# victorramirez952/tomography_3d_reconstructor

Hardware: AMD Instinct MI355X
Metric: Mvoxels/s (SDF+MC) on 1024^3 ellipsoid stack; achieved HBM GB/s vs peak (higher is better)
Workload: dtype f64

## Files before the change

### include/tomo_hip.h

```cpp
#ifndef TOMO_HIP_H
#define TOMO_HIP_H

#include <stddef.h>
#include <stdint.h>

#ifdef __cplusplus
extern "C" {
#endif

#define TOMO_OK 0
#define TOMO_E_ARG (-1)
#define TOMO_E_LAUNCH (-2)
#define TOMO_E_SIZE (-3)
#define TOMO_E_WORKSPACE (-4)

int tomo_abi_version(void);
const char *tomo_error_string(int code);
int tomo_host_mc_cell(const float *h_v, double iso, int8_t *h_tris, int *h_uses_centre);
double tomo_host_mc_edge_offset(double va, double vb);
void tomo_host_mc_centre_offset(const double *h_v8, double *h_out3);

int tomo_host_checksum(const void *h_data, int64_t nbytes, int nthreads, uint64_t *h_out);
int tomo_host_checksum_impl(const void *h_data, int64_t nbytes, int nthreads, int impl, uint64_t *h_out);
int64_t tomo_host_checksum_chunk_bytes(void);
// ... 106 lines not shown
                   const double *xt, double r2, int level, int32_t *map, void *workspace, int64_t workspace_bytes, void *stream);
int tomo_edt_threshold_masked(const uint64_t *sites, int nz, int ny, int nx, const double *zt, const double *yt, const double *xt,
                              int inside, double r2, int keep_less, const uint64_t *mask, uint64_t *out, void *workspace,
                              int64_t workspace_bytes, void *stream);
int tomo_edt_thickness_finish(int32_t *map, const uint64_t *bits, int nz, int ny, int nx, const float *values, int levels,
                              int64_t *counts, void *stream);
int tomo_pack_threshold(const uint8_t *grey, uint64_t *bits, int nz, int ny, int nx, int threshold, void *stream);
int tomo_obj_write(const char *path, const void *vertices, int vertex_is_double, int64_t nv, const int64_t *faces,
                   int64_t nf, int nthreads);
int tomo_obj_block_format(int kind, const void *h_rows, int64_t n, int nthreads, void **h_block, int64_t *h_nbytes);
int tomo_obj_block_pwrite(const char *path, int64_t offset, const void *h_block);
void tomo_obj_block_free(void *h_block);

int tomo_extend_bits(const uint64_t *bits, uint64_t *ext, int nz, int ny, int nx, int pad, void *stream);
int tomo_field_fill(const uint64_t *ext, float *field, int nz, int ny, int nx, int pad, int gaussian,
                    unsigned long long *signs, uint8_t *gcls, void *stream);
int tomo_field_fill_bits(const uint64_t *bits, float *field, int nz, int ny, int nx, int pad, unsigned long long *signs,
                         uint8_t *gcls, void *stream);
int64_t tomo_field_span_bytes(int nz, int ny, int nx, int pad);
int tomo_field_fill_bits_sparse(const uint64_t *bits, float *field, int nz, int ny, int nx, int pad, unsigned long long *signs,
                                uint8_t *gcls, uint8_t *span_ws, void *stream);
int64_t tomo_sign_rows(int Ny);
int64_t tomo_sign_buffer_words(int Nz, int Ny, int Nx, int xorg);
int tomo_field_signs(const float *field, int Nz, int Ny, int Nx, int64_t pitch, int xorg, double iso, int z_begin,
                     int z_end, unsigned long long *signs, uint8_t *gcls, void *stream);

int tomo_mc_classify(const unsigned long long *signs, const uint8_t *gcls, int Nz, int Ny, int Nx, int xorg,
                     unsigned long long *seg_act, uint32_t *seg_cnt, void *stream);
int tomo_mc_scan_segments(const uint32_t *seg_cnt, int64_t nseg, uint32_t *seg_aoff, unsigned long long *totals,
                          void *workspace, int64_t workspace_bytes, void *stream);
int64_t tomo_mc_scan_workspace_bytes(int64_t n);
int tomo_mc_scan(const uint32_t *counts, int64_t n, uint32_t *off_a, uint32_t *off_b, uint32_t *nz_ids,
                 unsigned long long *totals, void *workspace, int64_t workspace_bytes, void *stream);
int tomo_mc_list(int Nz, int Ny, int Nx, int xorg, const uint32_t *seg_aoff, const unsigned long long *seg_act,
                 unsigned long long *vox_key, void *stream);
int tomo_mc_eval(const float *field, int Nz, int Ny, int Nx, int64_t pitch, int xorg, double iso,
                 const unsigned long long *vox_key, int64_t na, uint32_t *vox_counts, uint8_t *vox_flags, void *stream);
int tomo_mc_list_capped(int Nz, int Ny, int Nx, int xorg, const uint32_t *seg_aoff, const unsigned long long *seg_act,
                        unsigned long long *vox_key, int64_t cap, void *stream);
int tomo_mc_eval_capped(const float *field, int Nz, int Ny, int Nx, int64_t pitch, int xorg, double iso,
                        const unsigned long long *vox_key, int64_t cap, const unsigned long long *na_dev,
                        uint32_t *vox_counts, uint8_t *vox_flags, void *stream);
int tomo_mc_emit(const float *field, int Nz, int Ny, int Nx, int64_t pitch, int xorg, double iso,
                 const unsigned long long *vox_key, int64_t na, const unsigned long long *seg_act,
                 const uint32_t *seg_aoff, const uint32_t *vox_voff, const uint32_t *vox_foff, const uint8_t *vox_flags,
                 int z_offset, unsigned long long *vkey, float *vpos, int32_t *faces, unsigned long long *totals,
                 void *stream);

int tomo_mc_first_touch(const float *field, int Nz, int Ny, int Nx, int64_t pitch, int xorg, double iso,
                        const unsigned long long *vox_key, int64_t na, const unsigned long long *seg_act,
                        const uint32_t *seg_aoff, const uint32_t *vox_voff, const uint8_t *vox_flags, int mode,
                        uint32_t *created, const uint32_t *base, int32_t *ft_rank, unsigned long long *totals, void *stream);

int tomo_mc3_list(int Nz, int Ny, int Nx, int xorg, const uint32_t *seg_cnt, const unsigned long long *seg_act,
                  uint32_t *seg_blk, uint32_t *seg_aoff, unsigned long long *vox_key, int64_t cap, unsigned long long *tot,
                  void *stream);
int tomo_mc3_eval(const float *field, int Nz, int Ny, int Nx, int64_t pitch, int xorg, double iso,
                  const unsigned long long *vox_key, int64_t cap, const unsigned long long *tot, int z_offset,
                  uint32_t *vox_loc, int32_t *vox_til, uint8_t *vox_flags, uint16_t *vox_used, float *vox_f3, float *vox_c3,
                  uint32_t *blk3, void *stream);
int64_t tomo_mc3_slice_table_words(int Nz, int Ny);
int64_t tomo_mc3_sort_segments(int Nz, int Ny);
int tomo_mc3_scan(int Nz, int Ny, int Nx, int xorg, const uint32_t *seg_aoff, const uint32_t *vox_loc, int64_t cap,
                  uint32_t *blk3, uint32_t *slice_tab, unsigned long long *tot, int64_t cap_v, int64_t cap_f, void *stream);
int tomo_mc3_vertices(int Nz, int Ny, int Nx, int xorg, const unsigned long long *vox_key, int64_t cap,
                      const unsigned long long *tot, const uint32_t *vox_loc, const uint8_t *vox_flags, const float *vox_f3,
                      const float *vox_c3, const uint32_t *blk3, const uint32_t *slice_tab, int z_offset, int shift,
                      const double *cum, int64_t ncum, const double *adj, int64_t nadj, float mm_y, float mm_x, float *vrec,
                      uint32_t *keys, uint32_t *idx, void *stream);
int64_t tomo_mc3_sort_workspace_bytes(int64_t cap_v, int64_t nseg);
int tomo_mc3_sort_rank_top(const float *vrec, uint32_t *keys, uint32_t *idx, int64_t cap_v, int Nz, int Ny, const uint32_t *slice_tab,
                           unsigned long long *tot, float *uniq, int32_t *table, void *workspace, int64_t workspace_bytes,
                           float z_top, void *stream);
int tomo_mc3_sort_rank_fused(const float *vrec, const uint32_t *keys, int64_t cap_v, int Nz, int Ny, uint32_t *slice_tab,
                             unsigned long long *tot, float *uniq, int32_t *table, float z_top, void *stream);
int tomo_mc3_faces(int Nz, int Ny, int Nx, int xorg, const unsigned long long *vox_key, int64_t cap, unsigned long long *tot,
                   const unsigned long long *seg_act, const uint32_t *seg_aoff, const uint32_t *vox_loc, const int32_t *vox_til,
                   const uint16_t *vox_used, const uint32_t *blk3, const int32_t *table, int64_t *faces, int64_t cap_f,
                   void *stream);

int tomo_vertex_finalize(float *vpos, int64_t nv, int shift, const double *cum, int64_t ncum,
                         const double *adj, int64_t nadj, float mm_y, float mm_x, void *stream);
int64_t tomo_mesh_unique_workspace_bytes(int64_t nv);
int tomo_mesh_unique(const float *vpos, int64_t nv, float *uniq, int32_t *rank, unsigned long long *totals,
                     void *workspace, int64_t workspace_bytes, void *stream);
int tomo_mesh_lookup(const float *uniq, int64_t nu, const float *query, int64_t nq, int32_t *out,
                     unsigned long long *missing, void *stream);
int tomo_slab_top_rows(const float *uniq, const unsigned long long *tot, int64_t cap_v, int64_t cap, float *msg, void *stream);
int tomo_slab_lookup(const float *uniq, const unsigned long long *tot, int64_t cap_v, const float *msg, int64_t cap,
                     int32_t *out, unsigned long long *missing, void *stream);
int tomo_slab_summary(const unsigned long long *tot, int64_t cap_v, const float *msg_in, unsigned long long *missing,
                      int64_t cap_top, int64_t caller_flags, int64_t *out, void *stream);
int tomo_slab_lookup_summary(const float *uniq, const unsigned long long *tot, int64_t cap_v, const float *msg, int64_t cap,
                             int32_t *out, int64_t cap_top, int64_t caller_flags, unsigned long long *scratch, int64_t *summary,
                             void *stream);
int tomo_mc3_faces_slab(int Nz, int Ny, int Nx, int xorg, const unsigned long long *vox_key, int64_t cap, unsigned long long *tot,
                        const unsigned long long *seg_act, const uint32_t *seg_aoff, const uint32_t *vox_loc, const int32_t *vox_til,
                        const uint16_t *vox_used, const uint32_t *blk3, const int32_t *table, int64_t *faces, int64_t cap_f,
                        const int64_t *gathered, int rank, int world, const int32_t *ids_next, int64_t cap_top, int64_t cap_v,
                        void *stream);
int tomo_mesh_volume_area(const float *verts, const int64_t *faces, int64_t nf, double *out, void *stream);

int tomo_layer_colors(const void *verts, int is_f64, int64_t nv, int64_t stride, double start1, double end1, int enable1,
                      double start2, double end2, int enable2, uint8_t *rgba, void *stream);
int64_t tomo_mesh_edge_table_bytes(int64_t nf);
int tomo_mesh_edges(const int64_t *faces, int64_t nf, int64_t nv, void *table, int64_t table_bytes, unsigned long long *counters,
// ... 25 lines not shown
```

### tomography_3d_reconstructor_amd/_lib.py

```python
import ctypes
import os
import subprocess

_HERE = os.path.dirname(os.path.abspath(__file__))
SO_PATH = os.environ.get("TOMO_LIB") or os.path.join(_HERE, "libtomo_hip.so")
CSRC = os.path.join(_HERE, "csrc")

_c_i = ctypes.c_int
_c_i64 = ctypes.c_int64
_c_p = ctypes.c_void_p
_c_d = ctypes.c_double
_c_f = ctypes.c_float

SIGNATURES = {
    "tomo_abi_version": (_c_i, []),
    "tomo_error_string": (ctypes.c_char_p, [_c_i]),
    "tomo_host_mc_cell": (_c_i, [_c_p, _c_d, _c_p, _c_p]),
    "tomo_host_mc_edge_offset": (_c_d, [_c_d, _c_d]),
    "tomo_host_mc_centre_offset": (None, [_c_p, _c_p]),
    "tomo_host_checksum": (_c_i, [_c_p, _c_i64, _c_i, _c_p]),
    "tomo_host_checksum_impl": (_c_i, [_c_p, _c_i64, _c_i, _c_i, _c_p]),
    "tomo_host_checksum_chunk_bytes": (_c_i64, []),
    "tomo_host_checksum_part": (_c_i, [_c_p, _c_i64, _c_i64, _c_i, _c_i, _c_p]),
    "tomo_host_checksum_fold": (_c_i, [_c_p, _c_i64, _c_i64, _c_p]),
# ... 39 lines not shown
    "tomo_cc_seam_union": (_c_i, [_c_p, _c_i, _c_i, _c_i, _c_p, _c_i64, _c_p, _c_p, _c_p, _c_p, _c_p, _c_p, _c_i64, _c_i64, _c_i64, _c_p,
                                  _c_p, _c_p]),
    "tomo_cc_merge_tables": (_c_i, [_c_p, _c_i, _c_i64, _c_i64, _c_p, _c_i64, _c_i64, _c_i64, _c_p, _c_p, _c_p, _c_p, _c_p, _c_p]),
    "tomo_cc_local_maps": (_c_i, [_c_p, _c_p, _c_p, _c_p, _c_i64, _c_i64, _c_i64, _c_i64, _c_i, _c_p, _c_p, _c_p]),
    "tomo_cc_filter_map": (_c_i, [_c_p, _c_i, _c_i, _c_i, _c_p, _c_i64, _c_p, _c_p, _c_p, _c_p, _c_i64, _c_p, _c_p]),
    "tomo_cc_expand_map": (_c_i, [_c_p, _c_i, _c_i, _c_i, _c_p, _c_i64, _c_p, _c_p, _c_p, _c_p, _c_i64, _c_p, _c_p]),
    "tomo_edt_workspace_bytes": (_c_i64, [_c_i, _c_i, _c_i, _c_i64]),
    "tomo_edt_chunk_columns": (_c_i64, [_c_i, _c_i, _c_i, _c_i64]),
    "tomo_edt_distance": (_c_i, [_c_p, _c_i, _c_i, _c_i, _c_p, _c_p, _c_p, _c_i, _c_p, _c_p, _c_i64, _c_p]),
    "tomo_edt_threshold": (_c_i, [_c_p, _c_i, _c_i, _c_i, _c_p, _c_p, _c_p, _c_i, _c_d, _c_i, _c_p, _c_p, _c_i64, _c_p]),
    "tomo_edt_argmax": (_c_i, [_c_p, _c_i, _c_i, _c_i, _c_p, _c_p, _c_p, _c_i, _c_p, _c_p, _c_i64, _c_p]),
    "tomo_edt_squared": (_c_i, [_c_p, _c_i, _c_i, _c_i, _c_p, _c_p, _c_p, _c_i, _c_p, _c_p, _c_i64, _c_p]),
    "tomo_edt_at_least": (_c_i, [_c_p, _c_p, _c_i, _c_i, _c_i, _c_d, _c_p, _c_p]),
    "tomo_edt_cover": (_c_i, [_c_p, _c_p, _c_i, _c_i, _c_i, _c_p, _c_p, _c_p, _c_d, _c_i, _c_p, _c_p, _c_i64, _c_p]),
    "tomo_edt_threshold_masked": (_c_i, [_c_p, _c_i, _c_i, _c_i, _c_p, _c_p, _c_p, _c_i, _c_d, _c_i, _c_p, _c_p, _c_p, _c_i64, _c_p]),
    "tomo_edt_thickness_finish": (_c_i, [_c_p, _c_p, _c_i, _c_i, _c_i, _c_p, _c_i, _c_p, _c_p]),
    "tomo_pack_threshold": (_c_i, [_c_p, _c_p, _c_i, _c_i, _c_i, _c_i, _c_p]),
    "tomo_obj_write": (_c_i, [ctypes.c_char_p, _c_p, _c_i, _c_i64, _c_p, _c_i64, _c_i]),
    "tomo_obj_block_format": (_c_i, [_c_i, _c_p, _c_i64, _c_i, ctypes.POINTER(_c_p), ctypes.POINTER(_c_i64)]),
    "tomo_obj_block_pwrite": (_c_i, [ctypes.c_char_p, _c_i64, _c_p]),
    "tomo_obj_block_free": (None, [_c_p]),
    "tomo_fill_holes_slice": (_c_i, [_c_p, _c_i, _c_i, _c_i, _c_i, _c_p, _c_p]),
    "tomo_fill_holes_ends": (_c_i, [_c_p, _c_i, _c_i, _c_i, _c_p, _c_p]),
    "tomo_pack_close_ends": (_c_i, [_c_p, _c_p, _c_i, _c_i, _c_i, _c_p, _c_p]),
    "tomo_pack_bits_pair": (_c_i, [_c_p, _c_p, _c_i, _c_p, _c_p, _c_i, _c_i, _c_i, _c_p]),
    "tomo_slab_edges": (_c_i, [_c_p, _c_p, _c_i, _c_i, _c_i, _c_i, _c_p, _c_p, _c_i, _c_i, _c_p, _c_p, _c_p, _c_i, _c_p, _c_p, _c_p, _c_p,
                               _c_i, _c_p, _c_p]),
    "tomo_pack_close_range": (_c_i, [_c_p, _c_p, _c_i, _c_i, _c_i, _c_i, _c_i, _c_p, _c_p, _c_i, _c_i, _c_p]),
    "tomo_close_ends_workspace_words": (_c_i64, [_c_i, _c_i, _c_i]),
    "tomo_close_ends_scan": (_c_i, [_c_p, _c_i, _c_i, _c_i, _c_p, _c_p]),
    "tomo_close_ends_gp": (_c_i, [_c_p, _c_i, _c_i, _c_i, _c_p, _c_p, _c_p]),
    "tomo_morph_fused": (_c_i, [_c_p, _c_p, _c_i, _c_i, _c_i, ctypes.c_uint32, _c_i, _c_p]),
    "tomo_smooth": (_c_i, [_c_p, _c_p, _c_i, _c_i, _c_i, _c_i, _c_i, _c_p]),
    "tomo_extend_bits": (_c_i, [_c_p, _c_p, _c_i, _c_i, _c_i, _c_i, _c_p]),
    "tomo_field_fill": (_c_i, [_c_p, _c_p, _c_i, _c_i, _c_i, _c_i, _c_i, _c_p, _c_p, _c_p]),
    "tomo_field_fill_bits": (_c_i, [_c_p, _c_p, _c_i, _c_i, _c_i, _c_i, _c_p, _c_p, _c_p]),
    "tomo_field_span_bytes": (_c_i64, [_c_i, _c_i, _c_i, _c_i]),
    "tomo_field_fill_bits_sparse": (_c_i, [_c_p, _c_p, _c_i, _c_i, _c_i, _c_i, _c_p, _c_p, _c_p, _c_p]),
    "tomo_sign_rows": (_c_i64, [_c_i]),
    "tomo_sign_buffer_words": (_c_i64, [_c_i, _c_i, _c_i, _c_i]),
    "tomo_field_signs": (_c_i, [_c_p, _c_i, _c_i, _c_i, _c_i64, _c_i, _c_d, _c_i, _c_i, _c_p, _c_p, _c_p]),
    "tomo_mc_classify": (_c_i, [_c_p, _c_p, _c_i, _c_i, _c_i, _c_i, _c_p, _c_p, _c_p]),
    "tomo_mc_scan_segments": (_c_i, [_c_p, _c_i64, _c_p, _c_p, _c_p, _c_i64, _c_p]),
    "tomo_mc_scan_workspace_bytes": (_c_i64, [_c_i64]),
    "tomo_mc_scan": (_c_i, [_c_p, _c_i64, _c_p, _c_p, _c_p, _c_p, _c_p, _c_i64, _c_p]),
    "tomo_mc_list": (_c_i, [_c_i, _c_i, _c_i, _c_i, _c_p, _c_p, _c_p, _c_p]),
    "tomo_mc_eval": (_c_i, [_c_p, _c_i, _c_i, _c_i, _c_i64, _c_i, _c_d, _c_p, _c_i64, _c_p, _c_p, _c_p]),
    "tomo_mc_list_capped": (_c_i, [_c_i, _c_i, _c_i, _c_i, _c_p, _c_p, _c_p, _c_i64, _c_p]),
    "tomo_mc_eval_capped": (_c_i, [_c_p, _c_i, _c_i, _c_i, _c_i64, _c_i, _c_d, _c_p, _c_i64, _c_p, _c_p, _c_p, _c_p]),
    "tomo_mc_emit": (_c_i, [_c_p, _c_i, _c_i, _c_i, _c_i64, _c_i, _c_d, _c_p, _c_i64, _c_p, _c_p, _c_p, _c_p, _c_p, _c_i, _c_p,
                            _c_p, _c_p, _c_p, _c_p]),
    "tomo_mc_first_touch": (_c_i, [_c_p, _c_i, _c_i, _c_i, _c_i64, _c_i, _c_d, _c_p, _c_i64, _c_p, _c_p, _c_p, _c_p, _c_i, _c_p,
                                   _c_p, _c_p, _c_p, _c_p]),
    "tomo_mc3_list": (_c_i, [_c_i, _c_i, _c_i, _c_i, _c_p, _c_p, _c_p, _c_p, _c_p, _c_i64, _c_p, _c_p]),
    "tomo_mc3_eval": (_c_i, [_c_p, _c_i, _c_i, _c_i, _c_i64, _c_i, _c_d, _c_p, _c_i64, _c_p, _c_i, _c_p, _c_p, _c_p, _c_p, _c_p,
                             _c_p, _c_p, _c_p]),
    "tomo_mc3_slice_table_words": (_c_i64, [_c_i, _c_i]),
    "tomo_mc3_sort_segments": (_c_i64, [_c_i, _c_i]),
    "tomo_mc3_scan": (_c_i, [_c_i, _c_i, _c_i, _c_i, _c_p, _c_p, _c_i64, _c_p, _c_p, _c_p, _c_i64, _c_i64, _c_p]),
    "tomo_mc3_vertices": (_c_i, [_c_i, _c_i, _c_i, _c_i, _c_p, _c_i64, _c_p, _c_p, _c_p, _c_p, _c_p, _c_p, _c_p, _c_i, _c_i,
                                 _c_p, _c_i64, _c_p, _c_i64, _c_f, _c_f, _c_p, _c_p, _c_p, _c_p]),
    "tomo_mc3_sort_workspace_bytes": (_c_i64, [_c_i64, _c_i64]),
    "tomo_mc3_sort_rank_top": (_c_i, [_c_p, _c_p, _c_p, _c_i64, _c_i, _c_i, _c_p, _c_p, _c_p, _c_p, _c_p, _c_i64, _c_f, _c_p]),
    "tomo_mc3_sort_rank_fused": (_c_i, [_c_p, _c_p, _c_i64, _c_i, _c_i, _c_p, _c_p, _c_p, _c_p, _c_f, _c_p]),
    "tomo_mc3_faces": (_c_i, [_c_i, _c_i, _c_i, _c_i, _c_p, _c_i64, _c_p, _c_p, _c_p, _c_p, _c_p, _c_p, _c_p, _c_p, _c_p, _c_i64, _c_p]),
    "tomo_vertex_finalize": (_c_i, [_c_p, _c_i64, _c_i, _c_p, _c_i64, _c_p, _c_i64, _c_f, _c_f, _c_p]),
    "tomo_mesh_unique_workspace_bytes": (_c_i64, [_c_i64]),
    "tomo_mesh_unique": (_c_i, [_c_p, _c_i64, _c_p, _c_p, _c_p, _c_p, _c_i64, _c_p]),
    "tomo_mesh_lookup": (_c_i, [_c_p, _c_i64, _c_p, _c_i64, _c_p, _c_p, _c_p]),
    "tomo_slab_top_rows": (_c_i, [_c_p, _c_p, _c_i64, _c_i64, _c_p, _c_p]),
    "tomo_slab_lookup": (_c_i, [_c_p, _c_p, _c_i64, _c_p, _c_i64, _c_p, _c_p, _c_p]),
    "tomo_slab_summary": (_c_i, [_c_p, _c_i64, _c_p, _c_p, _c_i64, _c_i64, _c_p, _c_p]),
    "tomo_slab_lookup_summary": (_c_i, [_c_p, _c_p, _c_i64, _c_p, _c_i64, _c_p, _c_i64, _c_i64, _c_p, _c_p, _c_p]),
    "tomo_mc3_faces_slab": (_c_i, [_c_i, _c_i, _c_i, _c_i, _c_p, _c_i64, _c_p, _c_p, _c_p, _c_p, _c_p, _c_p, _c_p, _c_p, _c_p, _c_i64,
                                   _c_p, _c_i, _c_i, _c_p, _c_i64, _c_i64, _c_p]),
    "tomo_mesh_volume_area": (_c_i, [_c_p, _c_p, _c_i64, _c_p, _c_p]),
    "tomo_layer_colors": (_c_i, [_c_p, _c_i, _c_i64, _c_i64, _c_d, _c_d, _c_i, _c_d, _c_d, _c_i, _c_p, _c_p]),
    "tomo_mesh_edge_table_bytes": (_c_i64, [_c_i64]),
    "tomo_mesh_edges": (_c_i, [_c_p, _c_i64, _c_i64, _c_p, _c_i64, _c_p, _c_p]),
    "tomo_mesh_seam_edges": (_c_i, [_c_p, _c_i64, _c_i64, _c_i64, _c_p, _c_i64, _c_p, _c_p]),
    "tomo_mesh_seam_merge": (_c_i, [_c_p, _c_i64, _c_i64, _c_p, _c_i64, _c_p, _c_p]),
    "tomo_mesh_orient_workspace_bytes": (_c_i64, [_c_i64]),
    "tomo_mesh_orient": (_c_i, [_c_p, _c_i64, _c_i64, _c_p, _c_i64, _c_p, _c_p, _c_p]),
    "tomo_mesh_signed_volume": (_c_i, [_c_p, _c_p, _c_i64, _c_p, _c_p, _c_p]),
    "tomo_glb_pack_faces": (_c_i, [_c_p, _c_i64, _c_p, _c_p, _c_p, _c_i, _c_p]),
    "tomo_glb_pack_positions": (_c_i, [_c_p, _c_i, _c_i64, _c_p, _c_p, _c_p]),
    "tomo_mesh_vertex_normals_workspace_bytes": (_c_i64, [_c_i64, _c_i64]),
    "tomo_mesh_vertex_normals": (_c_i, [_c_p, _c_i64, _c_p, _c_i, _c_i64, _c_p, _c_i64, _c_p, _c_p, _c_p]),
    "tomo_mesh_vertex_normals_seeded": (_c_i, [_c_p, _c_i64, _c_p, _c_i, _c_i64, _c_p, _c_i64, _c_p, _c_p, _c_p, _c_i64, _c_p, _c_i64,
                                              _c_i, _c_p]),
}

_LIB = None


class TomoError(RuntimeError):
    pass


class TomoUnavailable(TomoError):
    """No MI355X visible / libtomo_hip.so not built.  The one failure the drop-in classes never turn into the
    reference's `return None`: there is no CPU fallback to hide behind."""


def build(force=False):
    srcs = [os.path.join(CSRC, f) for f in os.listdir(CSRC) if f.endswith((".hip", ".h", ".cpp", "Makefile"))]
# ... 30 lines not shown
```

### tomography_3d_reconstructor_amd/csrc/mc.hip

```cpp
#include <cstring>
#include <cstdlib>
#include "tomo_common.h"
#include <rocprim/rocprim.hpp>

#define MC_LUT_QUAL __device__ const
#define MC_FN __device__ static inline
#include "mc_cell.h"

#define SEG 256
#define KEY_XBITS 20
static_assert(KEY_XBITS + 2 == TOMO_KEY_ROW_SHIFT, "key layout shared with mesh.hip");

struct McGrid {
    int Nz, Ny, Nx;
    int64_t pitch;
    int xorg;
    int segs_per_row;
    double iso;
};

typedef float float4u __attribute__((ext_vector_type(4), aligned(4)));
typedef float float2u __attribute__((ext_vector_type(2), aligned(4)));
typedef float float3u __attribute__((ext_vector_type(3), aligned(4)));
typedef int int3u __attribute__((ext_vector_type(3), aligned(4)));
// ... 808 lines not shown
                                                           const u64 *__restrict__ vox_key, int64_t cap,
                                                           const u64 *__restrict__ tot, int z_offset,
                                                           u32 *__restrict__ vox_loc, int32_t *__restrict__ vox_til,
                                                           uint8_t *__restrict__ vox_flags, uint16_t *__restrict__ vox_used,
                                                           float *__restrict__ vox_f3, float *__restrict__ vox_c3,
                                                           u32 *__restrict__ blk3, int64_t nblk)
{
    __shared__ u32 wsum[4];
    const int lane = threadIdx.x & 63, w = threadIdx.x >> 6;
    const int64_t i = (int64_t)blockIdx.x * MC3_BLK + threadIdx.x;
    const u64 na = tot[0];
    const bool live = i < cap && (u64)i < na && na <= (u64)cap;
    u32 packed = 0;
    if (live) {
        Cell c;
        load_cell(field, g, vox_key[i], c);
        int ntri = 0;
        int32_t til = 0;
        u32 used = 0;
        if (c.cell_ok && c.index != 0 && c.index != 255) {
            const McTiling t = mc_cell_tiling(c.v, c.index);
            ntri = t.ntri;
            if (t.centre) c.flags |= 8;
            til = (int32_t)(((intptr_t)t.tris - (intptr_t)LUT_TILING1) * 16 + ntri);
            const int ix = c.index;
#define BICH(a, b) ((u32)(((ix >> (a)) ^ (ix >> (b))) & 1))
            used = BICH(0, 1) | BICH(1, 2) << 1 | BICH(2, 3) << 2 | BICH(3, 0) << 3 | BICH(4, 5) << 4 | BICH(5, 6) << 5 | BICH(6, 7) << 6 |
                   BICH(7, 4) << 7 | BICH(0, 4) << 8 | BICH(1, 5) << 9 | BICH(2, 6) << 10 | BICH(3, 7) << 11 | (t.centre ? 1u << 12 : 0u);
#undef BICH
            if (ntri == 0) used = 0;
        }
        const int Zg = c.Z + z_offset;
        float3u f3;
        f3.x = (float)((double)Zg + mc_edge_offset(c.v[0], c.v[4]));
        f3.y = (float)((double)c.Y + mc_edge_offset(c.v[0], c.v[3]));
        f3.z = (float)((double)c.X + mc_edge_offset(c.v[0], c.v[1]));
        *(float3u *)(vox_f3 + 3 * i) = f3;
        if (c.flags & 8) {
            double ox, oy, oz;
            mc_centre_offset(c.v, &ox, &oy, &oz);
            *(float3u *)(vox_c3 + 3 * i) = (float3u){(float)((double)Zg + oz), (float)((double)c.Y + oy), (float)((double)c.X + ox)};
        }
        vox_til[i] = til;
        vox_flags[i] = (uint8_t)c.flags;
        vox_used[i] = (uint16_t)used;
        packed = (u32)__popc(c.flags & 3) | ((u32)__popc(c.flags & 12) << 10) | ((u32)ntri << 20);
    }
    const u32 inc = wave_inclusive_scan(packed);
    if (lane == 63) wsum[w] = inc;
    __syncthreads();
    u32 ex = inc - packed;
    for (int k = 0; k < w; k++) ex += wsum[k];
    if (i < cap) vox_loc[i] = ex;
    if (threadIdx.x == MC3_BLK - 1) {
        const u32 sum = ex + packed;
        blk3[blockIdx.x] = MC3_LOC_A(sum);
        blk3[nblk + blockIdx.x] = MC3_LOC_B(sum);
        blk3[2 * nblk + blockIdx.x] = MC3_LOC_T(sum);
    }
}

__global__ __launch_bounds__(1024) void mc3_scan_kernel(const McGrid g, const u32 *__restrict__ seg_aoff,
                                                        const u32 *__restrict__ vox_loc, int64_t cap, u32 *__restrict__ blk3,
                                                        int64_t nblk, u32 *__restrict__ slice_tab, u64 *__restrict__ tot,
                                                        int64_t cap_v, int64_t cap_f)
{
    __shared__ u32 lds[3 * 16 + 3];
    u64 totals[3];
    scan_small_inplace<3>(blk3, nblk, nblk, totals, lds);
    const u64 na = tot[0];
    const u64 totA64 = totals[0], totB64 = totals[1], totT64 = totals[2];
    const u32 totA = (u32)totA64, totB = (u32)totB64;
    const int Nz = g.Nz;
    u32 *sliceA = slice_tab, *sliceB = slice_tab + (Nz + 1);
    const int64_t segs_per_slice = (int64_t)g.Ny * g.segs_per_row;
    const bool fits = na <= (u64)cap;
    for (int Z = threadIdx.x; Z <= Nz; Z += 1024) {
        u32 a = totA, b = totB;
        if (Z < Nz && fits) {
            const u64 s = seg_aoff[(int64_t)Z * segs_per_slice];
            if (s < na) {
                const u32 l = vox_loc[s];
                a = blk3[s >> 8] + MC3_LOC_A(l);
                b = blk3[nblk + (s >> 8)] + MC3_LOC_B(l);
            }
        }
        sliceA[Z] = a;
        sliceB[Z] = b;
    }
    u64 ov = 0;
    if (totA64 + totB64 > (u64)cap_v) ov |= 2ull;
    if (totT64 > (u64)cap_f) ov |= 4ull;
    if (!fits) ov |= 1ull;
    if (threadIdx.x == 0) {
        tot[1] = totA64 + totB64;
        tot[2] = totT64;
        if (ov) atomicOr((unsigned long long *)&tot[3], (unsigned long long)ov);
    }
}

__global__ __launch_bounds__(256) void mc3_bands_kernel(const McGrid g, const u32 *__restrict__ seg_aoff,
                                                        const u32 *__restrict__ vox_loc, const u32 *__restrict__ blk3,
                                                        int64_t nblk, u32 *__restrict__ slice_tab, const u64 *__restrict__ tot)
{
    const int Nz = g.Nz, NB = TOMO_SORT_NB(g.Ny);
    const int64_t nseg = (int64_t)(NB + 1) * Nz, i = (int64_t)blockIdx.x * blockDim.x + threadIdx.x;
    const u32 *sliceA = slice_tab, *sliceB = slice_tab + (Nz + 1);
    u32 *offsets = slice_tab + 2 * (Nz + 1), *merge3 = offsets + nseg + 1;
    const bool ov = tot[3] != 0;
    const u64 na = tot[0];
    if (i == nseg) {
        offsets[nseg] = ov ? 0u : sliceA[Nz] + sliceB[Nz];
        merge3[0] = ov ? 0u : sliceA[1] + sliceB[0];
        merge3[1] = ov ? 0u : sliceA[1] + sliceB[1];
        merge3[2] = ov ? 0u : sliceA[Nz >= 2 ? 2 : 1] + sliceB[1];
        merge3[3] = 0u;
        return;
    }
    if (i > nseg) return;
    const int Z = (int)(i / (NB + 1)), b = (int)(i - (int64_t)Z * (NB + 1));
    u32 o = 0u;
    if (!ov) {
        if (b == NB) {
            o = sliceA[Z + 1] + sliceB[Z];
        } else {
            const u64 s = seg_aoff[((int64_t)Z * g.Ny + (int64_t)b * tomo_sort_band(g.Ny)) * g.segs_per_row];
            const u32 a = s < na ? blk3[s >> 8] + MC3_LOC_A(vox_loc[s]) : sliceA[Nz];
            o = a + sliceB[Z];
        }
    }
    offsets[i] = o;
}

struct Mc3Final {
    const double *cum, *adj;
    int64_t ncum, nadj;
    int shift;
    float mm_y, mm_x;
};

__device__ static inline void mc3_put_vertex(float z, float y, float x, u32 id, u32 dest, bool between, const Mc3Final &fin,
                                             float4 *__restrict__ vrec, u32 *__restrict__ keys, u32 *__restrict__ idx)
{
    if (fin.shift) { z -= 1.0f; y -= 1.0f; x -= 1.0f; }
    if (fin.nadj > 0) {
        if (z < 0.0f) z = 0.0f;
        else if ((double)z >= (double)(fin.ncum - 1)) z = (float)fin.cum[fin.ncum - 1];
// ... 134 lines not shown
            if (sl >= MC3_FWIN) continue;
            int32_t tv[3];
#pragma unroll
            for (int j = 0; j < 3; j++) {
                const int ed = tris[3 * tI + j];
                int32_t v = id0;
                v = ed == 1 ? id1 : v; v = ed == 2 ? id2 : v; v = ed == 3 ? id3 : v; v = ed == 4 ? id4 : v;
                v = ed == 5 ? id5 : v; v = ed == 6 ? id6 : v; v = ed == 7 ? id7 : v; v = ed == 8 ? id8 : v;
                v = ed == 9 ? id9 : v; v = ed == 10 ? id10 : v; v = ed == 11 ? id11 : v; v = ed == 12 ? id12 : v;
                tv[j] = v;
            }
            sf[3 * sl] = tv[2]; sf[3 * sl + 1] = tv[1]; sf[3 * sl + 2] = tv[0];
            degen += (tv[0] == tv[1] || tv[1] == tv[2] || tv[0] == tv[2]) ? 1 : 0;
        }
        __syncthreads();
        const u32 n = 3u * (total - w0 < MC3_FWIN ? total - w0 : (u32)MC3_FWIN);
        int64_t *dst = faces + 3 * (int64_t)(fbase + w0);
        if constexpr (SLAB) {
            int64_t off_me = 0;
            for (int r = 0; r < sm.rank; ++r) off_me += sm.gathered[8 * r];
            const int64_t off_next = off_me + sm.gathered[8 * sm.rank];
            const bool ok = tot[1] <= (u64)sm.cap_v && tot[7] <= tot[1];
            const int64_t k = ok ? (int64_t)(tot[1] - tot[7]) : 0;
            for (u32 e = threadIdx.x; e < n; e += MC3_BLK) {
                const int64_t row = (int64_t)sf[e];
                const int64_t j = row - k;
                dst[e] = row < k ? row + off_me : off_next + ((sm.ids_next && j < sm.cap_top) ? (int64_t)sm.ids_next[j] : 0);
            }
        } else {
            for (u32 e = threadIdx.x; e < n; e += MC3_BLK) dst[e] = (int64_t)sf[e];
        }
        __syncthreads();
    }
    if (degen) atomicAdd((unsigned long long *)&tot[5], (unsigned long long)degen);
    if (bad) atomicAdd((unsigned long long *)&tot[6], 1ull);
}

TOMO_API int tomo_mc3_eval(const float *field, int Nz, int Ny, int Nx, int64_t pitch, int xorg, double iso,
                           const unsigned long long *vox_key, int64_t cap, const unsigned long long *tot, int z_offset,
                           uint32_t *vox_loc, int32_t *vox_til, uint8_t *vox_flags, uint16_t *vox_used, float *vox_f3,
                           float *vox_c3, uint32_t *blk3, void *stream)
{
    McGrid g;
    int rc = make_grid(g, field, Nz, Ny, Nx, pitch, xorg, iso);
    if (rc) return rc;
    if (!vox_key || !tot || !vox_loc || !vox_til || !vox_flags || !vox_used || !vox_f3 || !vox_c3 || !blk3 || cap <= 0) return TOMO_E_ARG;
    const int64_t nblk = ceil_div64(cap, MC3_BLK);
    if (nblk > 0x7fffffff) return TOMO_E_SIZE;
    hipLaunchKernelGGL(mc3_eval_kernel, dim3((unsigned)nblk), dim3(MC3_BLK), 0, (hipStream_t)stream, field, g, (const u64 *)vox_key,
                       cap, (const u64 *)tot, z_offset, vox_loc, vox_til, vox_flags, vox_used, vox_f3, vox_c3, blk3, nblk);
    return tomo_status();
}

TOMO_API int64_t tomo_mc3_sort_segments(int Nz, int Ny) { return (int64_t)(TOMO_SORT_NB(Ny) + 1) * Nz; }
TOMO_API int64_t tomo_mc3_slice_table_words(int Nz, int Ny) { return 2 * ((int64_t)Nz + 1) + tomo_mc3_sort_segments(Nz, Ny) + 1 + 3 + 8; }

TOMO_API int tomo_mc3_scan(int Nz, int Ny, int Nx, int xorg, const uint32_t *seg_aoff, const uint32_t *vox_loc, int64_t cap,
                           uint32_t *blk3, uint32_t *slice_tab, unsigned long long *tot, int64_t cap_v, int64_t cap_f,
                           void *stream)
{
    if (Nz < 2 || Ny < 2 || Nx < 2 || !seg_aoff || !vox_loc || !blk3 || !slice_tab || !tot || cap <= 0) return TOMO_E_ARG;
    if (cap_v >= 0x7fffffffll || cap_f >= 0x7fffffffll) return TOMO_E_SIZE;
    McGrid g; g.Nz = Nz; g.Ny = Ny; g.Nx = Nx; g.pitch = 0; g.xorg = xorg; g.iso = 0.0;
    g.segs_per_row = (int)tomo_mc_segments_per_row(Nx, xorg);
    hipLaunchKernelGGL(mc3_scan_kernel, dim3(1), dim3(1024), 0, (hipStream_t)stream, g, seg_aoff, vox_loc, cap, blk3,
                       ceil_div64(cap, MC3_BLK), slice_tab, (u64 *)tot, cap_v, cap_f);
    const int64_t nseg = tomo_mc3_sort_segments(Nz, Ny);
    if (nseg + 1 > 0x7fffffff) return TOMO_E_SIZE;
    hipLaunchKernelGGL(mc3_bands_kernel, dim3((unsigned)ceil_div64(nseg + 1, 256)), dim3(256), 0, (hipStream_t)stream, g, seg_aoff,
                       vox_loc, (const u32 *)blk3, ceil_div64(cap, MC3_BLK), slice_tab, (const u64 *)tot);
    return tomo_status();
}

TOMO_API int tomo_mc3_vertices(int Nz, int Ny, int Nx, int xorg, const unsigned long long *vox_key, int64_t cap,
                               const unsigned long long *tot, const uint32_t *vox_loc, const uint8_t *vox_flags,
                               const float *vox_f3, const float *vox_c3, const uint32_t *blk3, const uint32_t *slice_tab,
                               int z_offset, int shift, const double *cum, int64_t ncum, const double *adj, int64_t nadj,
                               float mm_y, float mm_x, float *vrec, uint32_t *keys, uint32_t *idx, void *stream)
{
    if (Nz < 2 || Ny < 2 || Nx < 2 || !vox_key || !tot || !vox_loc || !vox_flags || !vox_f3 || !vox_c3 || !blk3 || !slice_tab ||
        !vrec || !keys || cap <= 0 || (nadj > 0 && (!cum || !adj || ncum != nadj + 1)))
        return TOMO_E_ARG;
    McGrid g; g.Nz = Nz; g.Ny = Ny; g.Nx = Nx; g.pitch = 0; g.xorg = xorg; g.iso = 0.0;
    g.segs_per_row = (int)tomo_mc_segments_per_row(Nx, xorg);
    Mc3Final fin; fin.cum = cum; fin.adj = adj; fin.ncum = ncum; fin.nadj = nadj; fin.shift = shift; fin.mm_y = mm_y; fin.mm_x = mm_x;
    const int64_t nblk = ceil_div64(cap, MC3_BLK);
    hipLaunchKernelGGL(mc3_vertices_kernel, dim3((unsigned)nblk), dim3(MC3_BLK), 0, (hipStream_t)stream, g, (const u64 *)vox_key, cap,
                       (const u64 *)tot, vox_loc, vox_flags, vox_f3, vox_c3, blk3, nblk, slice_tab, z_offset, fin, (float4 *)vrec,
                       keys, idx);
    return tomo_status();
}

TOMO_API int tomo_mc3_faces(int Nz, int Ny, int Nx, int xorg, const unsigned long long *vox_key, int64_t cap,
                            unsigned long long *tot, const unsigned long long *seg_act, const uint32_t *seg_aoff,
                            const uint32_t *vox_loc, const int32_t *vox_til, const uint16_t *vox_used, const uint32_t *blk3,
                            const int32_t *table, int64_t *faces, int64_t cap_f, void *stream)
{
    if (Nz < 2 || Ny < 2 || Nx < 2 || !vox_key || !tot || !seg_act || !seg_aoff || !vox_loc || !vox_til || !vox_used || !blk3 || !table || !faces ||
        cap <= 0 || cap_f < 0)
        return TOMO_E_ARG;
    McGrid g; g.Nz = Nz; g.Ny = Ny; g.Nx = Nx; g.pitch = 0; g.xorg = xorg; g.iso = 0.0;
    g.segs_per_row = (int)tomo_mc_segments_per_row(Nx, xorg);
    const int64_t nblk = ceil_div64(cap, MC3_BLK);
    hipLaunchKernelGGL(mc3_faces_kernel<false>, dim3((unsigned)nblk), dim3(MC3_BLK), 0, (hipStream_t)stream, g, (const u64 *)vox_key, cap,
                       (u64 *)tot, (const u64 *)seg_act, seg_aoff, vox_loc, vox_til, vox_used, blk3, nblk, table, faces, cap_f,
                       Mc3SlabMap{nullptr, nullptr, 0, 0, 0});
    return tomo_status();
}

TOMO_API int tomo_mc3_faces_slab(int Nz, int Ny, int Nx, int xorg, const unsigned long long *vox_key, int64_t cap,
                                 unsigned long long *tot, const unsigned long long *seg_act, const uint32_t *seg_aoff,
                                 const uint32_t *vox_loc, const int32_t *vox_til, const uint16_t *vox_used, const uint32_t *blk3,
                                 const int32_t *table, int64_t *faces, int64_t cap_f, const int64_t *gathered, int rank, int world,
                                 const int32_t *ids_next, int64_t cap_top, int64_t cap_v, void *stream)
{
    if (Nz < 2 || Ny < 2 || Nx < 2 || !vox_key || !tot || !seg_act || !seg_aoff || !vox_loc || !vox_til || !vox_used || !blk3 || !table || !faces ||
        cap <= 0 || cap_f < 0 || !gathered || rank < 0 || rank >= world || cap_v < 1 || cap_top < 0)
        return TOMO_E_ARG;
    McGrid g; g.Nz = Nz; g.Ny = Ny; g.Nx = Nx; g.pitch = 0; g.xorg = xorg; g.iso = 0.0;
    g.segs_per_row = (int)tomo_mc_segments_per_row(Nx, xorg);
    const int64_t nblk = ceil_div64(cap, MC3_BLK);
    hipLaunchKernelGGL(mc3_faces_kernel<true>, dim3((unsigned)nblk), dim3(MC3_BLK), 0, (hipStream_t)stream, g, (const u64 *)vox_key, cap,
                       (u64 *)tot, (const u64 *)seg_act, seg_aoff, vox_loc, vox_til, vox_used, blk3, nblk, table, faces, cap_f,
// ... 4 lines not shown
```

### tomography_3d_reconstructor_amd/pipeline.py

```python
import math
import os
import threading
from dataclasses import dataclass

import numpy as np
import torch

from . import _lib


COUNTERS = dict.fromkeys(("na_hint_hit", "na_hint_miss", "mc3_hint_hit", "mc3_hint_miss", "mc3_sort_fused", "mc3_sort_library",
                          "mc3_exact", "mc3_general_unique", "mc3_degenerate", "components_label", "components_expand",
                          "components_filter", "slab_components_label", "slab_components_seam", "slab_components_merge",
                          "slab_components_expand", "slab_components_filter", "distance_transform", "distance_offset",
                          "components_measure", "components_zhist", "components_moments", "components_euler",
                          "components_cavities", "local_thickness", "opening_volume"), 0)
NA_HINTS = os.environ.get("TOMO_NA_HINTS", "1") not in ("", "0")
_NA_HINT = {}
LIST_LIMIT = 2 ** 31
MESH_LIMIT = 2 ** 31
PACK_CLOSE_FUSED = os.environ.get("TOMO_PACK_CLOSE", "1") not in ("", "0")
FIELD_FROM_BITS = True
FIELD_SPARSE = os.environ.get("TOMO_FIELD_SPARSE", "0") not in ("", "0")

# ... 1046 lines not shown
    def wait(self, timeout_s=None):
        if timeout_s is None:
            self._event.synchronize()
        else:
            wait_event(self._event, timeout_s, "the counters of a pass")
        out = self._host.tolist()
        PendingDownload._free[self._key].append(self._host)
        self._host = None
        return out


class Mc3Surface:

    def __init__(self, f, slice_depths, mm_per_pixel_y, mm_per_pixel_x, add_padding=True, z_offset=0, z_top=None, tot=None):
        self.field, self.z_offset = f, int(z_offset)
        self.z_top = float("nan") if z_top is None else float(z_top)
        self.hint_key = (f.Nz, f.Ny, f.Nx, self.z_offset)
        self._depth = _depth_args(slice_depths, add_padding, f.data.device)
        self._mm = (float(np.float32(mm_per_pixel_y)), float(np.float32(mm_per_pixel_x)))
        self.tot = torch.empty(8, dtype=torch.int64, device=f.data.device) if tot is None else tot
        self.uniq = self.table = self.faces_final = None
        self.nv = self.nf = self.na = 0
        self.deferred = False
        self._pending = None

    def classify(self):
        L, f, dev = _lib.lib(), self.field, self.field.data.device
        if f.signs is None or f.signs_level != 0.5:
            if f.sparse:
                raise _lib.TomoError("a sparse field holds floats only near the 0.5 surface")
            field_signs(f, 0.5)
        nseg = f.Nz * f.Ny * L.tomo_mc_segments_per_row(f.Nx, f.xorg)
        self.seg_act = torch.empty(nseg * 4, dtype=torch.int64, device=dev)
        self.seg_cnt = torch.empty(nseg, dtype=torch.int32, device=dev)
        _lib.check(L.tomo_mc_classify(_p(f.signs), _p(f.gcls), f.Nz, f.Ny, f.Nx, f.xorg, _p(self.seg_act), _p(self.seg_cnt), _stream()),
                   "tomo_mc_classify")
        self.seg_blk = torch.empty((nseg + 255) // 256, dtype=torch.int32, device=dev)
        self.seg_aoff = torch.empty(nseg + 1, dtype=torch.int32, device=dev)

    def build_list(self, cap):
        f, self.cap = self.field, cap
        self.vox_key = torch.empty(cap, dtype=torch.int64, device=f.data.device)
        _lib.check(_lib.lib().tomo_mc3_list(f.Nz, f.Ny, f.Nx, f.xorg, _p(self.seg_cnt), _p(self.seg_act), _p(self.seg_blk), _p(self.seg_aoff),
                                            _p(self.vox_key), cap, _p(self.tot), _stream()), "tomo_mc3_list")

    def eval_scan(self, cap_v, cap_f):
        L, f, cap, st, dev = _lib.lib(), self.field, self.cap, _stream(), self.field.data.device
        self.vox_loc = torch.empty(cap, dtype=torch.int32, device=dev)
        self.vox_til = torch.empty(cap, dtype=torch.int32, device=dev)
        self.vox_flags = torch.empty(cap, dtype=torch.uint8, device=dev)
        self.vox_used = torch.empty(cap, dtype=torch.int16, device=dev)
        self.vox_f3 = torch.empty(3 * cap, dtype=torch.float32, device=dev)
        self.vox_c3 = torch.empty(3 * cap, dtype=torch.float32, device=dev)
        self.blk3 = torch.empty(3 * ((cap + 255) // 256), dtype=torch.int32, device=dev)
        self.slice_tab = torch.empty(L.tomo_mc3_slice_table_words(f.Nz, f.Ny), dtype=torch.int32, device=dev)
        _lib.check(L.tomo_mc3_eval(_p(f.data), f.Nz, f.Ny, f.Nx, f.pitch, f.xorg, 0.5, _p(self.vox_key), cap, _p(self.tot), self.z_offset,
                                   _p(self.vox_loc), _p(self.vox_til), _p(self.vox_flags), _p(self.vox_used), _p(self.vox_f3),
                                   _p(self.vox_c3), _p(self.blk3), st), "tomo_mc3_eval")
        _lib.check(L.tomo_mc3_scan(f.Nz, f.Ny, f.Nx, f.xorg, _p(self.seg_aoff), _p(self.vox_loc), cap, _p(self.blk3), _p(self.slice_tab),
                                   _p(self.tot), cap_v, cap_f, st), "tomo_mc3_scan")

    def vertices_sort(self, cap_v):
        L, f, cap, tot, st, dev = _lib.lib(), self.field, self.cap, self.tot, _stream(), self.field.data.device
        cum_t, ncum, adj_t, nadj = self._depth
        self.cap_v = cap_v
        self.vrec = torch.empty((cap_v, 4), dtype=torch.float32, device=dev)
        keys = torch.empty(cap_v, dtype=torch.int32, device=dev)
        self.rows = torch.empty((cap_v, 3), dtype=torch.float32, device=dev)
        self.table = torch.empty(4 * cap, dtype=torch.int32, device=dev)
        fused = FUSED_SORT and not _MC3_LARGE.get(self.hint_key)
        idx = None if fused else torch.empty(cap_v, dtype=torch.int32, device=dev)
        _lib.check(L.tomo_mc3_vertices(f.Nz, f.Ny, f.Nx, f.xorg, _p(self.vox_key), cap, _p(tot), _p(self.vox_loc), _p(self.vox_flags),
                                       _p(self.vox_f3), _p(self.vox_c3), _p(self.blk3), _p(self.slice_tab), self.z_offset, 1, _p(cum_t), ncum,
                                       _p(adj_t), nadj, *self._mm, _p(self.vrec), _p(keys), _p(idx), st), "tomo_mc3_vertices")
        if fused:
            COUNTERS["mc3_sort_fused"] += 1
            _lib.check(L.tomo_mc3_sort_rank_fused(_p(self.vrec), _p(keys), cap_v, f.Nz, f.Ny, _p(self.slice_tab), _p(tot), _p(self.rows),
                                                  _p(self.table), self.z_top, st), "tomo_mc3_sort_rank_fused")
            return
        COUNTERS["mc3_sort_library"] += 1
        wsb = L.tomo_mc3_sort_workspace_bytes(cap_v, L.tomo_mc3_sort_segments(f.Nz, f.Ny))
        ws = torch.empty(wsb, dtype=torch.uint8, device=dev)
        _lib.check(L.tomo_mc3_sort_rank_top(_p(self.vrec), _p(keys), _p(idx), cap_v, f.Nz, f.Ny, _p(self.slice_tab), _p(tot), _p(self.rows),
                                            _p(self.table), _p(ws), wsb, self.z_top, st), "tomo_mc3_sort_rank_top")

    def enqueue(self, cap, cap_v, cap_f):
        self.build_list(cap)
        self.eval_scan(cap_v, cap_f)
        self.vertices_sort(cap_v)
        self.cap_f = cap_f

    def faces(self, table=None, again=False, slab_map=None):
        L = _lib.lib()
        f, st = self.field, _stream()
        tab = self.table if table is None else table
        if tab.dtype != torch.int32 or tab.numel() < 4 * self.cap:
            raise ValueError("table must be int32 with 4 entries per list position")
        if again:
            self.tot[5:7].zero_()
        faces = torch.empty((max(self.cap_f, 1), 3), dtype=torch.int64, device=tab.device)
        args = (f.Nz, f.Ny, f.Nx, f.xorg, _p(self.vox_key), self.cap, _p(self.tot), _p(self.seg_act), _p(self.seg_aoff), _p(self.vox_loc),
                _p(self.vox_til), _p(self.vox_used), _p(self.blk3), _p(tab), _p(faces), self.cap_f)
        if slab_map is not None:
            gathered, rank, world, ids_next, cap_top, cap_v = slab_map
            _lib.check(L.tomo_mc3_faces_slab(*args, _p(gathered), rank, world, _p(ids_next), cap_top, cap_v, st), "tomo_mc3_faces_slab")
        else:
            _lib.check(L.tomo_mc3_faces(*args, st), "tomo_mc3_faces")
# ... 396 lines not shown
```

Measured before the change: 699,700.

## Parallelize mc3 block-offset scan across many workgroups with packed block sums

The eval kernel now writes one packed per-block sum into a fourth region of blk3 instead of three separate unpacked values. The scan kernel, previously a single 1024-thread workgroup, becomes a multi-workgroup grid. Each workgroup recomputes the prefix of all earlier blocks by re-reading the packed sums, scans its own chunk, and fills only the slice-table entries that fall in its range. The aim is to stop a single workgroup serializing a scan over millions of blocks, at the cost of quadratic redundant prefix reads and a larger blk3 buffer.

```diff
diff --git a/include/tomo_hip.h b/include/tomo_hip.h
--- a/include/tomo_hip.h
+++ b/include/tomo_hip.h
@@ -182,6 +182,7 @@
                         const uint32_t *seg_aoff, const uint32_t *vox_voff, const uint8_t *vox_flags, int mode,
                         uint32_t *created, const uint32_t *base, int32_t *ft_rank, unsigned long long *totals, void *stream);
 
+int64_t tomo_mc3_blk3_words(int64_t cap);
 int tomo_mc3_list(int Nz, int Ny, int Nx, int xorg, const uint32_t *seg_cnt, const unsigned long long *seg_act,
                   uint32_t *seg_blk, uint32_t *seg_aoff, unsigned long long *vox_key, int64_t cap, unsigned long long *tot,
                   void *stream);
diff --git a/tomography_3d_reconstructor_amd/_lib.py b/tomography_3d_reconstructor_amd/_lib.py
--- a/tomography_3d_reconstructor_amd/_lib.py
+++ b/tomography_3d_reconstructor_amd/_lib.py
@@ -115,6 +115,7 @@
                             _c_p, _c_p, _c_p, _c_p]),
     "tomo_mc_first_touch": (_c_i, [_c_p, _c_i, _c_i, _c_i, _c_i64, _c_i, _c_d, _c_p, _c_i64, _c_p, _c_p, _c_p, _c_p, _c_i, _c_p,
                                    _c_p, _c_p, _c_p, _c_p]),
+    "tomo_mc3_blk3_words": (_c_i64, [_c_i64]),
     "tomo_mc3_list": (_c_i, [_c_i, _c_i, _c_i, _c_i, _c_p, _c_p, _c_p, _c_p, _c_p, _c_i64, _c_p, _c_p]),
     "tomo_mc3_eval": (_c_i, [_c_p, _c_i, _c_i, _c_i, _c_i64, _c_i, _c_d, _c_p, _c_i64, _c_p, _c_i, _c_p, _c_p, _c_p, _c_p, _c_p,
                              _c_p, _c_p, _c_p]),
diff --git a/tomography_3d_reconstructor_amd/csrc/mc.hip b/tomography_3d_reconstructor_amd/csrc/mc.hip
--- a/tomography_3d_reconstructor_amd/csrc/mc.hip
+++ b/tomography_3d_reconstructor_amd/csrc/mc.hip
@@ -884,47 +884,81 @@
     u32 ex = inc - packed;
     for (int k = 0; k < w; k++) ex += wsum[k];
     if (i < cap) vox_loc[i] = ex;
-    if (threadIdx.x == MC3_BLK - 1) {
-        const u32 sum = ex + packed;
-        blk3[blockIdx.x] = MC3_LOC_A(sum);
-        blk3[nblk + blockIdx.x] = MC3_LOC_B(sum);
-        blk3[2 * nblk + blockIdx.x] = MC3_LOC_T(sum);
-    }
-}
-
-__global__ __launch_bounds__(1024) void mc3_scan_kernel(const McGrid g, const u32 *__restrict__ seg_aoff,
-                                                        const u32 *__restrict__ vox_loc, int64_t cap, u32 *__restrict__ blk3,
-                                                        int64_t nblk, u32 *__restrict__ slice_tab, u64 *__restrict__ tot,
-                                                        int64_t cap_v, int64_t cap_f)
-{
-    __shared__ u32 lds[3 * 16 + 3];
-    u64 totals[3];
-    scan_small_inplace<3>(blk3, nblk, nblk, totals, lds);
+    if (threadIdx.x == MC3_BLK - 1) blk3[3 * nblk + blockIdx.x] = ex + packed;
+}
+
+#define MC3_SCAN_T 1024
+__global__ __launch_bounds__(MC3_SCAN_T) void mc3_scan_kernel(const McGrid g, const u32 *__restrict__ seg_aoff,
+                                                              const u32 *__restrict__ vox_loc, int64_t cap, u32 *__restrict__ blk3,
+                                                              int64_t nblk, u32 *__restrict__ slice_tab, u64 *__restrict__ tot,
+                                                              int64_t cap_v, int64_t cap_f)
+{
+    __shared__ u32 preA[MC3_SCAN_T], preB[MC3_SCAN_T], wfront[3][16], wown[3][16];
+    const int lane = threadIdx.x & 63, w = threadIdx.x >> 6;
+    const u32 *packed = blk3 + 3 * nblk;
+    const int64_t first = (int64_t)blockIdx.x * MC3_SCAN_T, b = first + threadIdx.x;
+    const u32 own = b < nblk ? packed[b] : 0u;
+    u32 f[3] = {0u, 0u, 0u};
+#pragma unroll 4
+    for (int64_t i = threadIdx.x; i < first; i += MC3_SCAN_T) {
+        const u32 v = packed[i];
+        f[0] += MC3_LOC_A(v); f[1] += MC3_LOC_B(v); f[2] += MC3_LOC_T(v);
+    }
+    const u32 v3[3] = {MC3_LOC_A(own), MC3_LOC_B(own), MC3_LOC_T(own)};
+    u32 inc[3];
+#pragma unroll
+    for (int k = 0; k < 3; k++) {
+        inc[k] = wave_inclusive_scan(v3[k]);
+        f[k] = wave_sum(f[k]);
+        if (lane == 63) { wown[k][w] = inc[k]; wfront[k][w] = f[k]; }
+    }
+    __syncthreads();
+    u64 front[3], totals[3];
+    u32 pre[3];
+#pragma unroll
+    for (int k = 0; k < 3; k++) {
+        u32 before = 0, all = 0;
+        front[k] = 0;
+#pragma unroll
+        for (int j = 0; j < 16; j++) {
+            front[k] += wfront[k][j];
+            if (j < w) before += wown[k][j];
+            all += wown[k][j];
+        }
+        totals[k] = front[k] + all;
+        pre[k] = (u32)front[k] + before + inc[k] - v3[k];
+        if (b < nblk) blk3[k * nblk + b] = pre[k];
+    }
+    preA[threadIdx.x] = pre[0];
+    preB[threadIdx.x] = pre[1];
+    __syncthreads();
+    const bool last = blockIdx.x == gridDim.x - 1;
     const u64 na = tot[0];
     const u64 totA64 = totals[0], totB64 = totals[1], totT64 = totals[2];
-    const u32 totA = (u32)totA64, totB = (u32)totB64;
     const int Nz = g.Nz;
     u32 *sliceA = slice_tab, *sliceB = slice_tab + (Nz + 1);
     const int64_t segs_per_slice = (int64_t)g.Ny * g.segs_per_row;
     const bool fits = na <= (u64)cap;
-    for (int Z = threadIdx.x; Z <= Nz; Z += 1024) {
-        u32 a = totA, b = totB;
-        if (Z < Nz && fits) {
-            const u64 s = seg_aoff[(int64_t)Z * segs_per_slice];
-            if (s < na) {
+    for (int Z = threadIdx.x; Z <= Nz; Z += MC3_SCAN_T) {
+        u64 s = na;
+        if (Z < Nz && fits) s = seg_aoff[(int64_t)Z * segs_per_slice];
+        if (s < na) {
+            const int64_t blk = (int64_t)(s >> 8) - first;
+            if (blk >= 0 && blk < MC3_SCAN_T) {
                 const u32 l = vox_loc[s];
-                a = blk3[s >> 8] + MC3_LOC_A(l);
-                b = blk3[nblk + (s >> 8)] + MC3_LOC_B(l);
+                sliceA[Z] = preA[blk] + MC3_LOC_A(l);
+                sliceB[Z] = preB[blk] + MC3_LOC_B(l);
             }
-        }
-        sliceA[Z] = a;
-        sliceB[Z] = b;
+        } else if (last) {
+            sliceA[Z] = (u32)totA64;
+            sliceB[Z] = (u32)totB64;
+        }
     }
     u64 ov = 0;
     if (totA64 + totB64 > (u64)cap_v) ov |= 2ull;
     if (totT64 > (u64)cap_f) ov |= 4ull;
     if (!fits) ov |= 1ull;
-    if (threadIdx.x == 0) {
+    if (last && threadIdx.x == 0) {
         tot[1] = totA64 + totB64;
         tot[2] = totT64;
         if (ov) atomicOr((unsigned long long *)&tot[3], (unsigned long long)ov);
@@ -1165,6 +1199,7 @@
     return tomo_status();
 }
 
+TOMO_API int64_t tomo_mc3_blk3_words(int64_t cap) { return 4 * ceil_div64(cap > 0 ? cap : 1, MC3_BLK); }
 TOMO_API int64_t tomo_mc3_sort_segments(int Nz, int Ny) { return (int64_t)(TOMO_SORT_NB(Ny) + 1) * Nz; }
 TOMO_API int64_t tomo_mc3_slice_table_words(int Nz, int Ny) { return 2 * ((int64_t)Nz + 1) + tomo_mc3_sort_segments(Nz, Ny) + 1 + 3 + 8; }
 
@@ -1176,12 +1211,13 @@
     if (cap_v >= 0x7fffffffll || cap_f >= 0x7fffffffll) return TOMO_E_SIZE;
     McGrid g; g.Nz = Nz; g.Ny = Ny; g.Nx = Nx; g.pitch = 0; g.xorg = xorg; g.iso = 0.0;
     g.segs_per_row = (int)tomo_mc_segments_per_row(Nx, xorg);
-    hipLaunchKernelGGL(mc3_scan_kernel, dim3(1), dim3(1024), 0, (hipStream_t)stream, g, seg_aoff, vox_loc, cap, blk3,
-                       ceil_div64(cap, MC3_BLK), slice_tab, (u64 *)tot, cap_v, cap_f);
+    const int64_t nblk = ceil_div64(cap, MC3_BLK);
+    hipLaunchKernelGGL(mc3_scan_kernel, dim3((unsigned)ceil_div64(nblk, MC3_SCAN_T)), dim3(MC3_SCAN_T), 0, (hipStream_t)stream, g,
+                       seg_aoff, vox_loc, cap, blk3, nblk, slice_tab, (u64 *)tot, cap_v, cap_f);
     const int64_t nseg = tomo_mc3_sort_segments(Nz, Ny);
     if (nseg + 1 > 0x7fffffff) return TOMO_E_SIZE;
     hipLaunchKernelGGL(mc3_bands_kernel, dim3((unsigned)ceil_div64(nseg + 1, 256)), dim3(256), 0, (hipStream_t)stream, g, seg_aoff,
-                       vox_loc, (const u32 *)blk3, ceil_div64(cap, MC3_BLK), slice_tab, (const u64 *)tot);
+                       vox_loc, (const u32 *)blk3, nblk, slice_tab, (const u64 *)tot);
     return tomo_status();
 }
 
diff --git a/tomography_3d_reconstructor_amd/pipeline.py b/tomography_3d_reconstructor_amd/pipeline.py
--- a/tomography_3d_reconstructor_amd/pipeline.py
+++ b/tomography_3d_reconstructor_amd/pipeline.py
@@ -1122,7 +1122,7 @@
         self.vox_used = torch.empty(cap, dtype=torch.int16, device=dev)
         self.vox_f3 = torch.empty(3 * cap, dtype=torch.float32, device=dev)
         self.vox_c3 = torch.empty(3 * cap, dtype=torch.float32, device=dev)
-        self.blk3 = torch.empty(3 * ((cap + 255) // 256), dtype=torch.int32, device=dev)
+        self.blk3 = torch.empty(L.tomo_mc3_blk3_words(cap), dtype=torch.int32, device=dev)
         self.slice_tab = torch.empty(L.tomo_mc3_slice_table_words(f.Nz, f.Ny), dtype=torch.int32, device=dev)
         _lib.check(L.tomo_mc3_eval(_p(f.data), f.Nz, f.Ny, f.Nx, f.pitch, f.xorg, 0.5, _p(self.vox_key), cap, _p(self.tot), self.z_offset,
                                    _p(self.vox_loc), _p(self.vox_til), _p(self.vox_flags), _p(self.vox_used), _p(self.vox_f3),
```

Result: no change. 699,200 (-0.1%).
